# Prachet-Dev-Singh/DenseCLIP_Vit_multimodal

Measured on AMD Instinct MI355X. Metric: images/sec (fwd+bwd) ViT-B/16 DenseCLIP @1024x2048, higher is better.
Workload: dtype bf16

## Files before the change

### denseclip_vit_multimodal_amd/csrc/gemm.hip

```cpp
#include <mutex>
#include <type_traits>

#include "common.h"

namespace {

constexpr int BM = 128, BN = 128, BK = 64;
constexpr int TILE_BYTES = 128 * BK * 2;
constexpr int STAGE_BYTES = 2 * TILE_BYTES;
constexpr int EP_LD = 68;
constexpr int SMEM_BYTES = 4 * 64 * EP_LD * 4 > 2 * STAGE_BYTES ? 4 * 64 * EP_LD * 4 : 2 * STAGE_BYTES;

template <typename T>
__device__ __forceinline__ void store8(T* p, const float* v, bool full, int rem) {
    if (full) {
        if constexpr (sizeof(T) == 4) {
            f32x4 a = {v[0], v[1], v[2], v[3]}, b = {v[4], v[5], v[6], v[7]};
            *(f32x4*)p = a;
            *(f32x4*)(p + 4) = b;
        } else {
            typedef T t8 __attribute__((ext_vector_type(8)));
            t8 x;
#pragma unroll
            for (int e = 0; e < 8; ++e) x[e] = (T)v[e];
// ... 1581 lines not shown
    const int HW = g.H * g.W;
    const float invHW = 1.0f / (float)HW, invW = 1.0f / (float)g.W;
#pragma unroll
    for (int i = 0; i < ROWS_INST; ++i) {
        const int inst = wave * ROWS_INST + i;
        int m = m0 + inst * (64 / CPR) + lane / CPR;
        m = m < M ? m : M - 1;
        const int b = fdiv(m, HW, invHW);
        const int p = m - b * HW;
        const int y = fdiv(p, g.W, invW);
        R.y[i] = y;
        R.x[i] = p - y * g.W;
        R.base[i] = (int64_t)b * g.bstride + g.off + (int64_t)p * g.ld;
    }
}

template <typename T, int ROWS_INST, int BKT>
__device__ __forceinline__ void stage_conv_rows(const T* __restrict__ X, const T* __restrict__ zero,
                                                const ConvRows<ROWS_INST, BKT>& R, const PixGeo g, int Cin, int dir,
                                                int k0, char* lds, int wave, int lane) {
    constexpr int CPR = BKT / 8;
    const int tap = k0 / Cin, ci = k0 - tap * Cin;
    const int dy = (tap / 3 - 1) * dir, dx = (tap % 3 - 1) * dir;
    const int64_t shift = ((int64_t)dy * g.W + dx) * g.ld + ci;
#pragma unroll
    for (int i = 0; i < ROWS_INST; ++i) {
        const int inst = wave * ROWS_INST + i;
        const int r = inst * (64 / CPR) + lane / CPR;
        const int c = (lane % CPR) ^ big_sw<BKT>(r);
        const int yy = R.y[i] + dy, xx = R.x[i] + dx;
        const bool ok = yy >= 0 && yy < g.H && xx >= 0 && xx < g.W;
        const T* src = ok ? X + R.base[i] + shift + c * 8 : zero + c * 8;
        __builtin_amdgcn_global_load_lds((const void*)src, LDS_PTR(lds + inst * 1024), 16, 0, 0);
    }
}

template <typename T, int ROWS_INST, int BKT>
__device__ __forceinline__ void stage_conv_rows_buf(const T* X, uint32_t xbytes, const ConvRows<ROWS_INST, BKT>& R,
                                                    const PixGeo g, int Cin, int dir, int k0, char* lds, int wave,
                                                    int lane) {
#if defined(__HIP_DEVICE_COMPILE__)
    constexpr int CPR = BKT / 8;
    const rsrc_t rs = make_rsrc(X, xbytes);
    const int tap = k0 / Cin, ci = k0 - tap * Cin;
    const int dy = (tap / 3 - 1) * dir, dx = (tap % 3 - 1) * dir;
    const int shift = (int)((((int64_t)dy * g.W + dx) * g.ld + ci) * (int64_t)sizeof(T));
#pragma unroll
    for (int i = 0; i < ROWS_INST; ++i) {
        const int inst = wave * ROWS_INST + i;
        const int r = inst * (64 / CPR) + lane / CPR;
        const int c = (lane % CPR) ^ big_sw<BKT>(r);
        const int yy = R.y[i] + dy, xx = R.x[i] + dx;
        const bool ok = yy >= 0 && yy < g.H && xx >= 0 && xx < g.W;
        const uint32_t voff = ok ? (uint32_t)((int64_t)R.base[i] * (int64_t)sizeof(T) + shift + c * 16) : 0xFFFFFFF0u;
        __builtin_amdgcn_raw_ptr_buffer_load_lds(rs, LDS_PTR(lds + inst * 1024), 16, voff, 0, 0, 0);
    }
#endif
}

template <typename T, int EPI, typename OutT, int BM, int BN, int WM, int WN, int STAGES>
__global__ __launch_bounds__(64 * WM * WN, 1) void conv_nt_kernel(
    const T* __restrict__ X, const T* __restrict__ zero, PixGeo g, int Cin, int dir, const T* __restrict__ Bw,
    int64_t ldb, int M, int N, int tiles_m, int tiles_n, const void* __restrict__ aux, int64_t ld_aux,
    void* __restrict__ C, int64_t ldc, int map_hw, int map_gap, int map_off, uint32_t xbytes) {
    constexpr int BKT = 64;
    typedef BigCfg<BM, BN, WM, WN, STAGES, BKT> Cfg;
    typedef typename Mfma<T>::frag frag;
    __shared__ __attribute__((aligned(16))) char smem[Cfg::SMEM];
    const int lane = threadIdx.x & 63;
    const int wave = threadIdx.x >> 6;
    const int wm = wave / WN, wn = wave % WN;
    const int l16 = lane & 15, lq = lane >> 4;

    const int t = xcd_remap(blockIdx.x, tiles_m * tiles_n);
    const int m0 = (t / tiles_n) * BM;
    const int n0 = (t % tiles_n) * BN;
    const int nk = 9 * Cin / BKT;

    ConvRows<Cfg::A_INST, BKT> R;
    conv_rows_init<T, Cfg::A_INST, BKT>(R, g, M, m0, wave, lane);
    f32x4 acc[Cfg::NB][Cfg::MB];
#pragma unroll
    for (int i = 0; i < Cfg::NB; ++i)
#pragma unroll
        for (int j = 0; j < Cfg::MB; ++j) acc[i][j] = f32x4{0.f, 0.f, 0.f, 0.f};

    uint32_t vb[Cfg::B_INST];
    rows_voff<T, Cfg::B_INST, BKT>(ldb, n0, N, wave, lane, vb);
    const uint32_t bbytes = (uint32_t)((int64_t)N * ldb * sizeof(T));
    auto stage = [&](int kt, int slot) {
        char* base = smem + slot * Cfg::STAGE_BYTES;
        if (xbytes) stage_conv_rows_buf<T, Cfg::A_INST, BKT>(X, xbytes, R, g, Cin, dir, kt * BKT, base, wave, lane);
        else stage_conv_rows<T, Cfg::A_INST, BKT>(X, zero, R, g, Cin, dir, kt * BKT, base, wave, lane);
        stage_rows_buf<T, Cfg::B_INST>(Bw, bbytes, vb, (uint32_t)(kt * BKT * sizeof(T)), base + Cfg::A_BYTES, wave);
    };
#pragma unroll
    for (int s = 0; s < STAGES - 1; ++s)
        if (s < nk) stage(s, s);
    for (int kt = 0; kt < nk; ++kt) {
        if (kt + STAGES - 2 <= nk - 1) wait_vmcnt<Cfg::G * (STAGES - 2)>();
        else wait_vmcnt<0>();
        __builtin_amdgcn_s_barrier();
        __builtin_amdgcn_sched_barrier(0);
        if (kt + STAGES - 1 < nk) stage(kt + STAGES - 1, (kt + STAGES - 1) % STAGES);
        const char* At = smem + (kt % STAGES) * Cfg::STAGE_BYTES;
        const char* Bt = At + Cfg::A_BYTES;
#pragma unroll
        for (int ks = 0; ks < BKT / 32; ++ks) {
            frag fb[Cfg::NB], fa[Cfg::MB];
            const int ch = ks * 4 + lq;
#pragma unroll
            for (int i = 0; i < Cfg::NB; ++i) fb[i] = big_frag<T, BKT>(Bt, wn * Cfg::WTN + i * 16 + l16, ch);
#pragma unroll
            for (int j = 0; j < Cfg::MB; ++j) fa[j] = big_frag<T, BKT>(At, wm * Cfg::WTM + j * 16 + l16, ch);
#pragma unroll
            for (int j = 0; j < Cfg::MB; ++j)
#pragma unroll
                for (int i = 0; i < Cfg::NB; ++i) acc[i][j] = Mfma16<T>::mma(fb[i], fa[j], acc[i][j]);
        }
        __builtin_amdgcn_sched_barrier(0);
    }
    big_epilogue<T, EPI, OutT, Cfg>(acc, smem, M, N, m0 + wm * Cfg::WTM, n0 + wn * Cfg::WTN, nullptr, aux, ld_aux, C,
                                     ldc, nullptr, 0, 0, 1.0f, map_hw, map_gap, map_off);
}

template <typename T, bool AD = false>
__device__ __forceinline__ void stage_tile_tn_conv(const T* __restrict__ X, const T* __restrict__ zero, const PixGeo g,
                                                   int tap, int ci0, int k0, int krows, char* lds_tile, int wave,
                                                   int lane) {
    const int HW = g.H * g.W;
    const float invHW = 1.0f / (float)HW, invW = 1.0f / (float)g.W;
    const int dy = tap / 3 - 1, dx = tap % 3 - 1;
#pragma unroll
    for (int i = 0; i < 4; ++i) {
        const int inst = wave * 4 + i;
        const int r = inst * 4 + (lane >> 4);
        const int pc = lane & 15;
        const int c = pc ^ ((r & 3) << 2);
        int m = k0 + r;
        const bool in_k = m < krows;
        m = in_k ? m : krows - 1;
        const int b = fdiv(m, HW, invHW);
        const int p = m - b * HW;
        const int y = fdiv(p, g.W, invW);
        const int yy = y + dy, xx = p - y * g.W + dx;
        const bool ok = in_k && yy >= 0 && yy < g.H && xx >= 0 && xx < g.W;
        const T* src = ok ? X + (int64_t)b * g.bstride + g.off + ((int64_t)yy * g.W + xx) * g.ld + ci0 + c * 8
                          : zero + (c & 7) * 8;
        if constexpr (AD) glds16_asm(src, lds_tile + inst * 1024);
        else __builtin_amdgcn_global_load_lds((const void*)src, LDS_PTR(lds_tile + inst * 1024), 16, 0, 0);
    }
}

template <typename T, bool AD = false>
__global__ __launch_bounds__(256, 2) void conv_wgrad_kernel(const T* __restrict__ dY, int64_t ldy,
                                                            const T* __restrict__ X, const T* __restrict__ zero,
                                                            PixGeo g, int Cin, int M, int N, int Kpix, int k_chunk,
                                                            int tiles_m, int tiles_n, float* __restrict__ C,
                                                            int64_t slab) {
    __shared__ __attribute__((aligned(16))) char smem[SMEM_BYTES];
    const int lane = threadIdx.x & 63;
    const int wave = threadIdx.x >> 6;
    const int wm = wave >> 1, wn = wave & 1;
    const int t = xcd_remap(blockIdx.x, tiles_m * tiles_n);
    const int m0 = (t / tiles_n) * BM;
    const int n0 = (t % tiles_n) * BN;
    const int tap = n0 / Cin, ci0 = n0 - tap * Cin;
    const int kbeg = blockIdx.y * k_chunk;
    int nk = k_chunk / BK;
    if (kbeg + nk * BK > Kpix) nk = (Kpix - kbeg + BK - 1) / BK;
    nk = nk < 0 ? 0 : nk;

    f32x16 acc[2][2];
#pragma unroll
    for (int i = 0; i < 2; ++i)
#pragma unroll
        for (int j = 0; j < 2; ++j)
#pragma unroll
            for (int e = 0; e < 16; ++e) acc[i][j][e] = 0.f;
    if (nk > 0) {
        stage_tile_tn<T>(dY, ldy, kbeg, Kpix, m0, M, smem, wave, lane);
        stage_tile_tn_conv<T>(X, zero, g, tap, ci0, kbeg, Kpix, smem + TILE_BYTES, wave, lane);
    }
    __syncthreads();
    for (int kt = 0; kt < nk; ++kt) {
        const int cur = kt & 1;
        const char* At = smem + cur * STAGE_BYTES;
        const char* Bt = At + TILE_BYTES;
        const int k0 = kbeg + kt * BK;
        if (kt + 1 < nk) {
            char* nxt = smem + (cur ^ 1) * STAGE_BYTES;
            stage_tile_tn<T, AD>(dY, ldy, k0 + BK, Kpix, m0, M, nxt, wave, lane);
            stage_tile_tn_conv<T, AD>(X, zero, g, tap, ci0, k0 + BK, Kpix, nxt + TILE_BYTES, wave, lane);
        }
#pragma unroll
        for (int s = 0; s < 4; ++s) {
            typename Mfma<T>::frag fa[2], fb[2];
#pragma unroll
            for (int i = 0; i < 2; ++i) fa[i] = tr_frag_tn<T>(Bt, s, wn * 64 + i * 32, lane);
#pragma unroll
            for (int j = 0; j < 2; ++j) fb[j] = tr_frag_tn<T>(At, s, wm * 64 + j * 32, lane);
#pragma unroll
            for (int i = 0; i < 2; ++i)
#pragma unroll
                for (int j = 0; j < 2; ++j) acc[i][j] = Mfma<T>::mma(fa[i], fb[j], acc[i][j]);
        }
        if constexpr (AD) {
            wait_vmcnt<0>();
            __builtin_amdgcn_s_barrier();
        } else {
            __syncthreads();
        }
    }
    if constexpr (AD) __syncthreads();
    gemm_epilogue<T, DCLIP_EPI_SPLITK, float>(acc, smem, M, N, m0, n0, nullptr, nullptr, 0, C, N, nullptr, 0, slab,
                                               1.0f);
}

const void* conv_zero_row() {
    static void* z = nullptr;
    if (!z) {
        if (hipMalloc(&z, 256) != hipSuccess) return nullptr;
        if (hipMemset(z, 0, 256) != hipSuccess) return nullptr;
    }
    return z;
}

float* tail_scratch(size_t floats) {
    static float* buf = nullptr;
    static size_t cap = 0;
    if (floats > cap) {
        if (buf) (void)hipFree(buf);
        buf = nullptr;
        cap = 0;
        if (hipMalloc(&buf, floats * sizeof(float)) != hipSuccess) return nullptr;
        cap = floats;
    }
    return buf;
}

template <typename T, int EPI, typename OutT>
__global__ __launch_bounds__(512) void gemm_tail16_kernel(const T* __restrict__ A, int64_t lda, const T* __restrict__ B,
                                                          int64_t ldb, int mt, int N, int K, int m0,
                                                          const float* __restrict__ bias, const void* __restrict__ aux,
                                                          int64_t ld_aux, void* __restrict__ C, int64_t ldc,
                                                          void* __restrict__ C2, int64_t ldc2, Alpha alpha_arg) {
    typedef typename Mfma<T>::frag frag;
    __shared__ float red[8][16][68];
    const int lane = threadIdx.x & 63, wave = threadIdx.x >> 6;
    const int l16 = lane & 15, lq = lane >> 4;
    const int n0 = blockIdx.x * 64;
    const int ks = K / 8, kbeg = wave * ks;
    const bool rowok = l16 < mt;
    const T* arow = A + (int64_t)(rowok ? l16 : 0) * lda + kbeg + 8 * lq;
    const T* brow = B + (int64_t)(n0 + l16) * ldb + kbeg + 8 * lq;
    f32x4 acc[4];
#pragma unroll
    for (int i = 0; i < 4; ++i) acc[i] = f32x4{0.f, 0.f, 0.f, 0.f};
    frag zf;
#pragma unroll
    for (int j = 0; j < 8; ++j) zf[j] = (T)0.f;
#pragma unroll 4
    for (int k = 0; k < ks; k += 32) {
        const frag a = rowok ? *(const frag*)(arow + k) : zf;
        frag b[4];
#pragma unroll
        for (int i = 0; i < 4; ++i) b[i] = *(const frag*)(brow + (int64_t)16 * i * ldb + k);
#pragma unroll
        for (int i = 0; i < 4; ++i) acc[i] = Mfma16<T>::mma(a, b[i], acc[i]);
    }
#pragma unroll
    for (int i = 0; i < 4; ++i)
#pragma unroll
        for (int e = 0; e < 4; ++e) red[wave][4 * lq + e][16 * i + l16] = acc[i][e];
    __syncthreads();
    const int t = threadIdx.x;
    if (t < 128) {
        const int r = t >> 3, cb = (t & 7) * 8;
        if (r < mt) {
            const float alpha = alpha_arg.get();
            float v[8];
#pragma unroll
            for (int e = 0; e < 8; ++e) {
                float sum = 0.f;
#pragma unroll
                for (int w = 0; w < 8; ++w) sum += red[w][r][cb + e];
                v[e] = sum * alpha;
            }
            epi_row8<T, EPI, OutT>(v, m0 + r, n0 + cb, N, bias, aux, ld_aux, C, ldc, C2, ldc2, 0);
        }
    }
}

template <typename T, int EPI, typename OutT>
__global__ __launch_bounds__(1024) void gemm_tail16x16_kernel(const T* __restrict__ A, int64_t lda,
                                                              const T* __restrict__ B, int64_t ldb, int mt, int N,
                                                              int W, int IT, int m0, const float* __restrict__ bias,
                                                              const void* __restrict__ aux, int64_t ld_aux,
                                                              void* __restrict__ C, int64_t ldc, void* __restrict__ C2,
                                                              int64_t ldc2, Alpha alpha_arg) {
    typedef typename Mfma<T>::frag frag;
    constexpr int ITMAX = 6;
    __shared__ float red[16][16][17];
    const int lane = threadIdx.x & 63, wave = threadIdx.x >> 6;
    const int l16 = lane & 15, lq = lane >> 4;
    const int n0 = blockIdx.x * 16;
    const int t = threadIdx.x;
    const int er = t >> 1, ecb = (t & 1) * 8;
    const bool epi = t < 2 * mt;
    float bv[8], pre[8];
#pragma unroll
    for (int e = 0; e < 8; ++e) bv[e] = pre[e] = 0.f;
    if (epi) {
        const int nb = n0 + ecb;
        if (bias != nullptr && EPI != DCLIP_EPI_GELU_BWD) load8<float>(bias + nb, bv, true, 8);
        if constexpr (EPI == DCLIP_EPI_STORE_SCALED) load8<float>((const float*)aux + nb, pre, true, 8);
        if constexpr (EPI == DCLIP_EPI_RESIDUAL)
            load8<float>((const float*)aux + (int64_t)(m0 + er) * ld_aux + nb, pre, true, 8);
        if constexpr (EPI == DCLIP_EPI_GELU_BWD) load8<T>((const T*)aux + (int64_t)(m0 + er) * ld_aux + nb, pre, true, 8);
    }
    const bool rowok = l16 < mt;
    const int kbeg = wave * IT * 32;
    const T* arow = A + (int64_t)(rowok ? l16 : 0) * lda + kbeg + 8 * lq;
    const T* brow = B + (int64_t)(n0 + l16) * ldb + kbeg + 8 * lq;
    frag zf;
#pragma unroll
    for (int j = 0; j < 8; ++j) zf[j] = (T)0.f;
    frag a[ITMAX], b[ITMAX];
#pragma unroll
    for (int it = 0; it < ITMAX; ++it) {
        if (it < IT) {
            a[it] = rowok ? *(const frag*)(arow + 32 * it) : zf;
            b[it] = *(const frag*)(brow + 32 * it);
        }
    }
    f32x4 acc = f32x4{0.f, 0.f, 0.f, 0.f};
#pragma unroll
    for (int it = 0; it < ITMAX; ++it)
        if (it < IT) acc = Mfma16<T>::mma(a[it], b[it], acc);
#pragma unroll
    for (int e = 0; e < 4; ++e) red[wave][4 * lq + e][l16] = acc[e];
    __syncthreads();
    if (epi) {
        const float alpha = alpha_arg.get();
        float v[8];
#pragma unroll
        for (int e = 0; e < 8; ++e) {
            float sum = 0.f;
            for (int w = 0; w < W; ++w) sum += red[w][er][ecb + e];
            v[e] = sum * alpha + bv[e];
        }
        const int64_t m = m0 + er;
        const int nb = n0 + ecb;
        if constexpr (EPI == DCLIP_EPI_STORE) {
            store8<OutT>((OutT*)C + m * ldc + nb, v, true, 8);
        } else if constexpr (EPI == DCLIP_EPI_STORE_SCALED) {
#pragma unroll
            for (int e = 0; e < 8; ++e) v[e] *= pre[e];
            store8<OutT>((OutT*)C + m * ldc + nb, v, true, 8);
        } else if constexpr (EPI == DCLIP_EPI_GELU) {
            float g[8];
#pragma unroll
            for (int e = 0; e < 8; ++e) {
                v[e] = (float)(OutT)v[e];
                g[e] = quick_gelu(v[e]);
            }
            if (C != nullptr) store8<OutT>((OutT*)C + m * ldc + nb, v, true, 8);
            store8<OutT>((OutT*)C2 + m * ldc2 + nb, g, true, 8);
        } else if constexpr (EPI == DCLIP_EPI_RESIDUAL) {
// ... 393 lines not shown
                             void* ws, void* C, int64_t ldc, float* colsum_a, void* stream) {
    const Alpha alpha(alpha_v, alpha_ptr);
    DCLIP_HOST_CHECK(ab_dt == DCLIP_BF16 || ab_dt == DCLIP_F16, "dclip_gemm_tn: operands must be f16/bf16");
    DCLIP_HOST_CHECK(M > 0 && N > 0 && K > 0 && M % 8 == 0 && N % 8 == 0,
                     "dclip_gemm_tn: M, N must be positive multiples of 8 (M=%lld N=%lld)", (long long)M, (long long)N);
    DCLIP_HOST_CHECK(splits >= 1 && K_pad >= K && K_pad % (BK * splits) == 0,
                     "dclip_gemm_tn: K_pad must be >= K and a multiple of 64*splits");
    DCLIP_HOST_CHECK(lda >= M && ldb >= N && lda % 8 == 0 && ldb % 8 == 0, "dclip_gemm_tn: bad leading dims");
    DCLIP_HOST_CHECK(((uintptr_t)A % 16) == 0 && ((uintptr_t)B % 16) == 0, "dclip_gemm_tn: A/B must be 16-byte aligned");
    DCLIP_HOST_CHECK(epilogue == DCLIP_EPI_STORE || epilogue == DCLIP_EPI_SPLITK,
                     "dclip_gemm_tn: epilogue must be STORE or SPLITK (f32 output)");
    DCLIP_HOST_CHECK(epilogue == DCLIP_EPI_STORE ? splits == 1 : ws != nullptr,
                     "dclip_gemm_tn: STORE needs splits == 1; SPLITK needs a workspace of splits*(M*N + M) f32");
    DCLIP_HOST_CHECK(ldc % 4 == 0, "dclip_gemm_tn: ldc %% 4 != 0");
    DCLIP_HOST_CHECK(K * lda * 2 < (1ll << 32) && K * ldb * 2 < (1ll << 32),
                     "dclip_gemm_tn: operands must stay below 4 GiB (buffer-load staging)");
    hipStream_t st = (hipStream_t)stream;
    const int tiles_m = (int)((M + BM - 1) / BM), tiles_n = (int)((N + BN - 1) / BN);
    const int k_chunk = (int)(K_pad / splits);
    dim3 grid(tiles_m * tiles_n, splits);
    const int tn_opt = dclip_option(DCLIP_OPT_GEMM_TN_TILE);
    const bool tn_pf = dclip_option(DCLIP_OPT_GEMM_KLOOP) == 1;
    const bool big = tn_opt != 1 && M >= 256 && N >= 256;
    const bool fused_cs =
        colsum_a && big && tn_opt != 2 && tn_opt != 3 && dclip_option(DCLIP_OPT_GEMM_TN_COLSUM) != 1;
    float* cs_sep = (colsum_a && !fused_cs && epilogue == DCLIP_EPI_SPLITK) ? (float*)ws + (int64_t)splits * M * N
                                                                           : nullptr;
    if (colsum_a && !fused_cs) {
        const int64_t rpb = cs_sep != nullptr ? K_pad / splits : K;
        dim3 cg((unsigned)((M + 63) / 64), (unsigned)(cs_sep != nullptr ? splits : 1));
        if (ab_dt == DCLIP_BF16)
            colsum_kernel<bf16><<<cg, 256, 0, st>>>((const bf16*)A, lda, K, (int)M, rpb, alpha, colsum_a, cs_sep);
        else colsum_kernel<f16><<<cg, 256, 0, st>>>((const f16*)A, lda, K, (int)M, rpb, alpha, colsum_a, cs_sep);
    }
#define TN_LAUNCH_V(T, EPI, OUT, AD)                                                                              \
    gemm_tn_kernel<T, EPI, float, AD><<<grid, 256, 0, st>>>((const T*)A, lda, (const T*)B, ldb, (int)M, (int)N,    \
                                                            (int)K, k_chunk, tiles_m, tiles_n, nullptr, OUT,         \
                                                            EPI == DCLIP_EPI_SPLITK ? N : ldc, (int64_t)M * N, alpha)
#define TN_LAUNCH(T, EPI, OUT)                                                                                    \
    do {                                                                                                          \
        if (tn_opt == 5) TN_LAUNCH_V(T, EPI, OUT, false);                                                         \
        else TN_LAUNCH_V(T, EPI, OUT, true);                                                                      \
    } while (0)
#define TN_BIG_V(T, EPI, OUT, BKT, STG, CS, NW, ...)                                                           \
    gemm_tn_big_kernel<T, EPI, BKT, STG, CS, NW, ##__VA_ARGS__><<<dim3(tm2 * tn2 * splits), 64 * NW, 0, st>>>( \
        (const T*)A, lda, (const T*)B, ldb, (int)M, (int)N, (int)K, k_chunk, tm2, tn2, OUT,                     \
        EPI == DCLIP_EPI_SPLITK ? N : ldc, (int64_t)M * N, alpha, EPI == DCLIP_EPI_SPLITK ? cs_part : colsum_a)
#define TN_BIG(T, EPI, OUT)                                                                                    \
    do {                                                                                                       \
        if (tn_opt == 2) TN_BIG_V(T, EPI, OUT, 32, 4, false, 8);                                               \
        else if (tn_opt == 3) TN_BIG_V(T, EPI, OUT, 32, 5, false, 8);                                          \
        else if (tn_opt == 4 && fused_cs) TN_BIG_V(T, EPI, OUT, 64, 2, true, 4);                               \
        else if (tn_opt == 4) TN_BIG_V(T, EPI, OUT, 64, 2, false, 4);                                          \
        else if (tn_opt == 5 && fused_cs) TN_BIG_V(T, EPI, OUT, 64, 2, true, 8);                               \
        else if (tn_opt == 5) TN_BIG_V(T, EPI, OUT, 64, 2, false, 8);                                          \
        else if (fused_cs && tn_pf) TN_BIG_V(T, EPI, OUT, 64, 2, true, 8, true, true);                         \
        else if (tn_pf) TN_BIG_V(T, EPI, OUT, 64, 2, false, 8, true, true);                                    \
        else if (fused_cs) TN_BIG_V(T, EPI, OUT, 64, 2, true, 8, false, true);                                 \
        else TN_BIG_V(T, EPI, OUT, 64, 2, false, 8, false, true);                                              \
    } while (0)
    const int tm2 = (int)((M + 255) / 256), tn2 = (int)((N + 255) / 256);
    float* cs_part = (fused_cs && epilogue == DCLIP_EPI_SPLITK) ? (float*)ws + (int64_t)splits * M * N : cs_sep;
    if (epilogue == DCLIP_EPI_STORE) {
        DCLIP_HOST_CHECK(bias == nullptr, "dclip_gemm_tn: bias only with SPLITK");
        if (big) {
            if (ab_dt == DCLIP_BF16) TN_BIG(bf16, DCLIP_EPI_STORE, C);
            else TN_BIG(f16, DCLIP_EPI_STORE, C);
        } else {
            if (ab_dt == DCLIP_BF16) TN_LAUNCH(bf16, DCLIP_EPI_STORE, C);
            else TN_LAUNCH(f16, DCLIP_EPI_STORE, C);
        }
    } else {
        if (big) {
            if (ab_dt == DCLIP_BF16) TN_BIG(bf16, DCLIP_EPI_SPLITK, ws);
            else TN_BIG(f16, DCLIP_EPI_SPLITK, ws);
        } else {
            if (ab_dt == DCLIP_BF16) TN_LAUNCH(bf16, DCLIP_EPI_SPLITK, ws);
            else TN_LAUNCH(f16, DCLIP_EPI_SPLITK, ws);
        }
        const int64_t total4 = M * (N / 4);
        int blocks = (int)((total4 + 255) / 256);
        blocks = blocks > 4096 ? 4096 : blocks;
        splitk_reduce_kernel<<<blocks, 256, 0, st>>>((const float*)ws, splits, M * N, (int)M, (int)N, bias,
                                                     (float*)C, ldc, cs_part, colsum_a);
    }
#undef TN_LAUNCH
#undef TN_LAUNCH_V
#undef TN_BIG
#undef TN_BIG_V
    DCLIP_LAUNCH_CHECK();
    return 0;
}

extern "C" int dclip_conv3x3(int mode, int ab_dt, const void* X, int64_t x_bstride, int64_t x_off, int64_t x_ld,
                             int B, int H, int W, int Cin, const void* Wt, int Nout, void* out, int out_dt,
                             int64_t out_ld, int out_gap, int out_off, int accumulate, void* stream) {
    DCLIP_HOST_CHECK(ab_dt == DCLIP_BF16 || ab_dt == DCLIP_F16, "dclip_conv3x3: operands must be f16/bf16");
    DCLIP_HOST_CHECK(mode == 0 || mode == 1, "dclip_conv3x3: mode 0 (forward) or 1 (input gradient)");
    DCLIP_HOST_CHECK(B > 0 && H > 0 && W > 0 && Cin > 0 && Nout > 0 && Cin % 64 == 0 && Nout % 8 == 0,
                     "dclip_conv3x3: Cin %% 64 == 0 and Nout %% 8 == 0 required (Cin=%d Nout=%d)", Cin, Nout);
    DCLIP_HOST_CHECK((int64_t)B * H * W < (1ll << 24), "dclip_conv3x3: too many pixels");
    DCLIP_HOST_CHECK(x_ld % 8 == 0 && x_bstride % 8 == 0 && x_off % 8 == 0 && x_ld >= Cin,
                     "dclip_conv3x3: input strides must be multiples of 8 elements");
    DCLIP_HOST_CHECK(((uintptr_t)X % 16) == 0 && ((uintptr_t)Wt % 16) == 0, "dclip_conv3x3: unaligned operands");
    DCLIP_HOST_CHECK(out_dt == ab_dt || out_dt == DCLIP_F32, "dclip_conv3x3: output must be f32 or the operand dtype");
    DCLIP_HOST_CHECK(!accumulate || out_dt == DCLIP_F32, "dclip_conv3x3: accumulate needs an f32 output");
    const void* zero = conv_zero_row();
    DCLIP_HOST_CHECK(zero != nullptr, "dclip_conv3x3: zero row allocation failed");
    hipStream_t st = (hipStream_t)stream;
    const PixGeo g{x_bstride, x_off, (int)x_ld, H, W};
    const int M = B * H * W;
    const int dir = mode == 0 ? 1 : -1;
    constexpr int TBM = 256, TBN = 128;
    const int tiles_m = (M + TBM - 1) / TBM, tiles_n = (Nout + TBN - 1) / TBN;
    const int map_hw = out_gap ? H * W : 0;
    const int64_t xext = ((int64_t)(B - 1) * x_bstride + x_off + (int64_t)H * W * x_ld) * 2;
    const uint32_t xbytes = xext < (1ll << 32) - 4096 ? (uint32_t)xext : 0u;
#define CONV_LAUNCH(T, EPI, OUTT)                                                                                    \
    conv_nt_kernel<T, EPI, OUTT, TBM, TBN, 4, 2, 3><<<tiles_m * tiles_n, 512, 0, st>>>(                             \
        (const T*)X, (const T*)zero, g, Cin, dir, (const T*)Wt, 9 * (int64_t)Cin, M, Nout, tiles_m, tiles_n, out,    \
        out_ld, out, out_ld, map_hw, out_gap, out_off, xbytes)
    if (ab_dt == DCLIP_BF16) {
        if (accumulate) CONV_LAUNCH(bf16, DCLIP_EPI_RESIDUAL, float);
        else if (out_dt == DCLIP_F32) CONV_LAUNCH(bf16, DCLIP_EPI_STORE, float);
        else CONV_LAUNCH(bf16, DCLIP_EPI_STORE, bf16);
    } else {
        if (accumulate) CONV_LAUNCH(f16, DCLIP_EPI_RESIDUAL, float);
        else if (out_dt == DCLIP_F32) CONV_LAUNCH(f16, DCLIP_EPI_STORE, float);
        else CONV_LAUNCH(f16, DCLIP_EPI_STORE, f16);
    }
#undef CONV_LAUNCH
    DCLIP_LAUNCH_CHECK();
    return 0;
}

extern "C" int dclip_conv3x3_wgrad(int ab_dt, const void* dY, int64_t ldy, int Nout, const void* X, int64_t x_bstride,
                                   int64_t x_off, int64_t x_ld, int B, int H, int W, int Cin, float* dW, void* ws,
                                   int splits, int oihw, const float* alpha_ptr, void* stream) {
    DCLIP_HOST_CHECK(ab_dt == DCLIP_BF16 || ab_dt == DCLIP_F16, "dclip_conv3x3_wgrad: operands must be f16/bf16");
    DCLIP_HOST_CHECK(Cin % 128 == 0 && Nout % 8 == 0 && Nout > 0 && ldy % 8 == 0 && ldy >= Nout,
                     "dclip_conv3x3_wgrad: Cin %% 128 == 0 and Nout %% 8 == 0 required");
    DCLIP_HOST_CHECK(x_ld % 8 == 0 && x_bstride % 8 == 0 && x_off % 8 == 0, "dclip_conv3x3_wgrad: bad strides");
    DCLIP_HOST_CHECK(splits >= 1 && ws != nullptr, "dclip_conv3x3_wgrad: workspace of splits * Nout * 9 * Cin f32");
    DCLIP_HOST_CHECK((int64_t)B * H * W < (1ll << 24), "dclip_conv3x3_wgrad: too many pixels");
    const void* zero = conv_zero_row();
    DCLIP_HOST_CHECK(zero != nullptr, "dclip_conv3x3_wgrad: zero row allocation failed");
    hipStream_t st = (hipStream_t)stream;
    const PixGeo g{x_bstride, x_off, (int)x_ld, H, W};
    const int Kpix = B * H * W;
    const int N = 9 * Cin;
    const int kp = (Kpix + 64 * splits - 1) / (64 * splits) * 64;
    const int tiles_m = (Nout + BM - 1) / BM, tiles_n = N / BN;
    dim3 grid(tiles_m * tiles_n, splits);
#define WG_LAUNCH(T, AD)                                                                                        \
    conv_wgrad_kernel<T, AD><<<grid, 256, 0, st>>>((const T*)dY, ldy, (const T*)X, (const T*)zero, g, Cin, Nout, N, \
                                                   Kpix, kp, tiles_m, tiles_n, (float*)ws, (int64_t)Nout * N)
    const bool ad = dclip_option(DCLIP_OPT_GEMM_TN_TILE) != 5;
    if (ab_dt == DCLIP_BF16) {
        if (ad) WG_LAUNCH(bf16, true);
        else WG_LAUNCH(bf16, false);
    } else {
        if (ad) WG_LAUNCH(f16, true);
        else WG_LAUNCH(f16, false);
    }
#undef WG_LAUNCH
    if (oihw || alpha_ptr != nullptr) {
        const int64_t total = (int64_t)Nout * Cin;
        const int blocks = (int)((total + 255) / 256 > 4096 ? 4096 : (total + 255) / 256);
        if (oihw) {
            conv_wgrad_reduce_oihw_kernel<<<blocks, 256, 0, st>>>((const float*)ws, splits, (int64_t)Nout * N, Nout, Cin,
                                                                  Alpha(1.f, alpha_ptr), dW);
            DCLIP_LAUNCH_CHECK();
            return 0;
        }
        DCLIP_HOST_CHECK(false, "dclip_conv3x3_wgrad: alpha_ptr needs the OIHW output");
    }
    const int64_t total4 = (int64_t)Nout * (N / 4);
    int blocks = (int)((total4 + 255) / 256);
    blocks = blocks > 4096 ? 4096 : blocks;
    splitk_reduce_kernel<<<blocks, 256, 0, st>>>((const float*)ws, splits, (int64_t)Nout * N, Nout, N, nullptr, dW,
                                                 N);
    DCLIP_LAUNCH_CHECK();
    return 0;
}
```

Measured before the change: 65.08.

## Carry pixel coordinates across K-steps in conv3x3 wgrad; add row-reuse kernel

The default conv3x3 weight-gradient path now keeps per-row pixel index, x coordinate and batch base in registers and advances them incrementally each K-step. This replaces the per-tile integer divisions used to compute im2col addresses. Separately, an opt-in kernel (option 7) builds one 17-row X tile per dy and derives all three dx taps from row-shifted LDS reads, masking image-edge columns. It uses a 3-stage pipeline with 512 threads. The carried path adds a vmcnt wait after the first stage, and its while-loop wrap only handles small strides cleanly.

```diff
diff --git a/denseclip_vit_multimodal_amd/csrc/gemm.hip b/denseclip_vit_multimodal_amd/csrc/gemm.hip
--- a/denseclip_vit_multimodal_amd/csrc/gemm.hip
+++ b/denseclip_vit_multimodal_amd/csrc/gemm.hip
@@ -1757,7 +1757,51 @@
     }
 }
 
-template <typename T, bool AD = false>
+struct TapRows {
+    int p[4], x[4];
+    int64_t base[4];
+};
+__device__ __forceinline__ void tap_rows_init(TapRows& R, const PixGeo g, int k0, int wave, int lane) {
+    const int HW = g.H * g.W;
+#pragma unroll
+    for (int i = 0; i < 4; ++i) {
+        const int m = k0 + (wave * 4 + i) * 4 + (lane >> 4);
+        const int b = m / HW;
+        R.p[i] = m - b * HW;
+        R.x[i] = R.p[i] % g.W;
+        R.base[i] = (int64_t)b * g.bstride + g.off;
+    }
+}
+template <typename T>
+__device__ __forceinline__ void stage_tile_tn_conv_carried(const T* __restrict__ X, const T* __restrict__ zero,
+                                                           const PixGeo g, int tap, int ci0, int k0, int krows,
+                                                           TapRows& R, char* lds_tile, int wave, int lane) {
+    const int HW = g.H * g.W, xstep = BK % g.W;
+    const int dy = tap / 3 - 1, dx = tap % 3 - 1;
+    const int plo = dy < 0 ? g.W : 0, phi = dy > 0 ? HW - g.W : HW;
+    const int xlo = dx < 0 ? 1 : 0, xhi = dx > 0 ? g.W - 1 : g.W;
+    const int shift = dy * g.W + dx;
+#pragma unroll
+    for (int i = 0; i < 4; ++i) {
+        const int inst = wave * 4 + i;
+        const int r = inst * 4 + (lane >> 4);
+        const int pc = lane & 15;
+        const int c = pc ^ ((r & 3) << 2);
+        const int p = R.p[i], x = R.x[i];
+        const bool ok = (k0 + r < krows) & (p >= plo) & (p < phi) & (x >= xlo) & (x < xhi);
+        const T* in = X + R.base[i] + (int64_t)(p + shift) * g.ld + ci0 + c * 8;
+        const T* src = ok ? in : zero + (c & 7) * 8;
+        glds16_asm(src, lds_tile + inst * 1024);
+        R.p[i] = p + BK;
+        R.x[i] = x + xstep >= g.W ? x + xstep - g.W : x + xstep;
+        while (R.p[i] >= HW) {
+            R.p[i] -= HW;
+            R.base[i] += g.bstride;
+        }
+    }
+}
+
+template <typename T, bool AD = false, bool CARRY = false>
 __global__ __launch_bounds__(256, 2) void conv_wgrad_kernel(const T* __restrict__ dY, int64_t ldy,
                                                             const T* __restrict__ X, const T* __restrict__ zero,
                                                             PixGeo g, int Cin, int M, int N, int Kpix, int k_chunk,
@@ -1783,9 +1827,16 @@
         for (int j = 0; j < 2; ++j)
 #pragma unroll
             for (int e = 0; e < 16; ++e) acc[i][j][e] = 0.f;
+    TapRows R;
+    if constexpr (CARRY) tap_rows_init(R, g, kbeg, wave, lane);
     if (nk > 0) {
         stage_tile_tn<T>(dY, ldy, kbeg, Kpix, m0, M, smem, wave, lane);
-        stage_tile_tn_conv<T>(X, zero, g, tap, ci0, kbeg, Kpix, smem + TILE_BYTES, wave, lane);
+        if constexpr (CARRY) {
+            stage_tile_tn_conv_carried<T>(X, zero, g, tap, ci0, kbeg, Kpix, R, smem + TILE_BYTES, wave, lane);
+            wait_vmcnt<0>();
+        } else {
+            stage_tile_tn_conv<T>(X, zero, g, tap, ci0, kbeg, Kpix, smem + TILE_BYTES, wave, lane);
+        }
     }
     __syncthreads();
     for (int kt = 0; kt < nk; ++kt) {
@@ -1796,7 +1847,9 @@
         if (kt + 1 < nk) {
             char* nxt = smem + (cur ^ 1) * STAGE_BYTES;
             stage_tile_tn<T, AD>(dY, ldy, k0 + BK, Kpix, m0, M, nxt, wave, lane);
-            stage_tile_tn_conv<T, AD>(X, zero, g, tap, ci0, k0 + BK, Kpix, nxt + TILE_BYTES, wave, lane);
+            if constexpr (CARRY)
+                stage_tile_tn_conv_carried<T>(X, zero, g, tap, ci0, k0 + BK, Kpix, R, nxt + TILE_BYTES, wave, lane);
+            else stage_tile_tn_conv<T, AD>(X, zero, g, tap, ci0, k0 + BK, Kpix, nxt + TILE_BYTES, wave, lane);
         }
 #pragma unroll
         for (int s = 0; s < 4; ++s) {
@@ -1820,6 +1873,194 @@
     if constexpr (AD) __syncthreads();
     gemm_epilogue<T, DCLIP_EPI_SPLITK, float>(acc, smem, M, N, m0, n0, nullptr, nullptr, 0, C, N, nullptr, 0, slab,
                                                1.0f);
+}
+
+constexpr bool CONV_WGRAD_ROWS_DEFAULT = false;
+constexpr bool CONV_WGRAD_CARRY_DEFAULT = true;
+constexpr int RW_A_BYTES = 64 * 256;
+constexpr int RW_X_PIECES = 17;
+constexpr int RW_STAGE_BYTES = RW_A_BYTES + RW_X_PIECES * 1024;
+constexpr int RW_STAGES = 3;
+constexpr int RW_EP_LD = 36;
+constexpr int RW_SMEM = RW_STAGES * RW_STAGE_BYTES > 8 * 64 * RW_EP_LD * 4 ? RW_STAGES * RW_STAGE_BYTES
+                                                                          : 8 * 64 * RW_EP_LD * 4;
+
+template <typename T>
+__device__ __forceinline__ typename Mfma<T>::frag tr_frag_rows(const char* img, int row0, int col_base, int lane) {
+    const int i = lane & 15, q = i >> 2, p = i & 3, g = lane >> 4, h = lane >> 5;
+    const int row = row0 + 8 * h + q;
+    const int col = col_base + (g & 1) * 16 + 4 * p;
+    typedef __attribute__((address_space(3))) i16x4 lds_i16x4;
+    auto off = [](int r, int c) { return r * 256 + (((c >> 3) ^ ((r & 3) << 2)) << 4) + ((c & 7) << 1); };
+    i16x4 lo = __builtin_amdgcn_ds_read_tr16_b64_v4i16((lds_i16x4*)(img + off(row, col)));
+    i16x4 hi = __builtin_amdgcn_ds_read_tr16_b64_v4i16((lds_i16x4*)(img + off(row + 4, col)));
+    typedef short s8 __attribute__((ext_vector_type(8)));
+    s8 v = __builtin_shufflevector(lo, hi, 0, 1, 2, 3, 4, 5, 6, 7);
+    return __builtin_bit_cast(typename Mfma<T>::frag, v);
+}
+
+template <typename F>
+__device__ __forceinline__ F zero_frag_rows(F f, uint32_t bits) {
+    typedef uint32_t u4 __attribute__((ext_vector_type(4)));
+    u4 v = __builtin_bit_cast(u4, f);
+#pragma unroll
+    for (int d = 0; d < 4; ++d) {
+        const uint32_t keep = ((bits >> (2 * d)) & 1u ? 0u : 0x0000FFFFu) | ((bits >> (2 * d + 1)) & 1u ? 0u : 0xFFFF0000u);
+        v[d] &= keep;
+    }
+    return __builtin_bit_cast(F, v);
+}
+
+template <typename T, int MJ>
+__global__ __launch_bounds__(512, 1) void conv_wgrad_rows_kernel(const T* __restrict__ dY, int64_t ldy,
+                                                                 const T* __restrict__ X, const T* __restrict__ zero,
+                                                                 PixGeo g, int Cin, int M, int N, int Kpix, int k_chunk,
+                                                                 int tiles_m, float* __restrict__ C, int64_t slab) {
+    typedef typename Mfma<T>::frag frag;
+    __shared__ __attribute__((aligned(16))) char smem[RW_SMEM];
+    const int lane = threadIdx.x & 63;
+    const int wave = __builtin_amdgcn_readfirstlane(threadIdx.x >> 6);
+    const int wm = wave >> 2, wq = wave & 3;
+    const int h = lane >> 5;
+    const int cb = Cin / 128;
+    const int t = xcd_remap(blockIdx.x, tiles_m * 3 * cb);
+    const int m0 = (t / (3 * cb)) * (64 * MJ);
+    const int rem = t % (3 * cb);
+    const int dy = rem / cb - 1, ci0 = (rem % cb) * 128;
+    const int W = g.W, HW = g.H * g.W;
+    const int kbeg = blockIdx.y * k_chunk;
+    int nk = k_chunk / BK;
+    if (kbeg + nk * BK > Kpix) nk = (Kpix - kbeg + BK - 1) / BK;
+    nk = nk < 0 ? 0 : nk;
+
+    f32x16 acc[3][MJ];
+#pragma unroll
+    for (int d = 0; d < 3; ++d)
+#pragma unroll
+        for (int j = 0; j < MJ; ++j)
+#pragma unroll
+            for (int e = 0; e < 16; ++e) acc[d][j][e] = 0.f;
+
+    const int lrow = lane >> 4, pc = lane & 15;
+    int xp[3];
+    int64_t xbase[3];
+#pragma unroll
+    for (int i = 0; i < 3; ++i) {
+        const int piece = i < 2 ? wave * 2 + i : 16;
+        const int m = kbeg - 1 + piece * 4 + lrow;
+        const int b = m >= 0 ? m / HW : -1;
+        xp[i] = m - b * HW;
+        xbase[i] = (int64_t)b * g.bstride + g.off;
+    }
+    int ks = kbeg;
+    const int plo = dy < 0 ? W : 0, phi = dy > 0 ? HW - W : HW;
+    auto stage = [&](int slot) {
+        char* At = smem + slot * RW_STAGE_BYTES;
+        char* Xt = At + RW_A_BYTES;
+#pragma unroll
+        for (int i = 0; i < 2; ++i) {
+            const int inst = wave * 2 + i;
+            const int r = inst * 4 + lrow;
+            const int c = pc ^ ((r & 3) << 2);
+            int gr = ks + r;
+            gr = gr < Kpix ? gr : Kpix - 1;
+            int gc = m0 + c * 8;
+            gc = gc + 8 <= M ? gc : M - 8;
+            glds16_asm(dY + (int64_t)gr * ldy + gc, At + inst * 1024);
+        }
+#pragma unroll
+        for (int i = 0; i < 3; ++i) {
+            const int piece = i < 2 ? wave * 2 + i : 16;
+            if (i < 2 || wave == 0) {
+                const int lr = piece * 4 + lrow;
+                const int c = pc ^ ((lr & 3) << 2);
+                const int m = ks - 1 + lr;
+                const bool ok = (m >= 0) & (m < Kpix) & (xp[i] >= plo) & (xp[i] < phi);
+                const T* in = X + xbase[i] + (int64_t)(xp[i] + dy * W) * g.ld + ci0 + c * 8;
+                const T* src = ok ? in : zero + (c & 7) * 8;
+                glds16_asm(src, Xt + piece * 1024);
+            }
+            xp[i] += BK;
+            while (xp[i] >= HW) {
+                xp[i] -= HW;
+                xbase[i] += g.bstride;
+            }
+        }
+        ks += BK;
+    };
+
+    if (nk > 0) stage(0);
+    if (nk > 1) stage(1);
+    int xk = kbeg % W;
+    const int xstep = BK % W;
+    int cur = 0, nxt = 2;
+    const int mc0 = (MJ == 2 ? 64 : 32) * wm;
+    for (int kt = 0; kt < nk; ++kt) {
+        if (kt + 1 < nk) wait_vmcnt<4>();
+        else wait_vmcnt<0>();
+        __builtin_amdgcn_s_barrier();
+        __builtin_amdgcn_sched_barrier(0);
+        if (kt + 2 < nk) stage(nxt);
+        const char* At = smem + cur * RW_STAGE_BYTES;
+        const char* Xt = At + RW_A_BYTES;
+        uint64_t mL = 0, mR = 0;
+        for (int r = xk == 0 ? 0 : W - xk; r <= BK; r += W) {
+            if (r < BK) mL |= 1ull << r;
+            if (r > 0) mR |= 1ull << (r - 1);
+        }
+        const bool edge = (mL | mR) != 0;
+#pragma unroll
+        for (int s = 0; s < 4; ++s) {
+            frag fa[3], fb[MJ];
+#pragma unroll
+            for (int j = 0; j < MJ; ++j) fb[j] = tr_frag_rows<T>(At, 16 * s, mc0 + 32 * j, lane);
+#pragma unroll
+            for (int d = 0; d < 3; ++d) fa[d] = tr_frag_rows<T>(Xt, 16 * s + d, 32 * wq, lane);
+            if (edge) {
+                fa[0] = zero_frag_rows(fa[0], (uint32_t)(mL >> (16 * s + 8 * h)) & 0xFFu);
+                fa[2] = zero_frag_rows(fa[2], (uint32_t)(mR >> (16 * s + 8 * h)) & 0xFFu);
+            }
+#pragma unroll
+            for (int d = 0; d < 3; ++d)
+#pragma unroll
+                for (int j = 0; j < MJ; ++j) acc[d][j] = Mfma<T>::mma(fa[d], fb[j], acc[d][j]);
+        }
+        __builtin_amdgcn_sched_barrier(0);
+        xk += xstep;
+        xk = xk >= W ? xk - W : xk;
+        cur = cur == 2 ? 0 : cur + 1;
+        nxt = nxt == 2 ? 0 : nxt + 1;
+    }
+    __syncthreads();
+
+    float* ep = (float*)smem + wave * (64 * RW_EP_LD);
+    const int l32 = lane & 31;
+    const int c4 = (lane & 7) * 4;
+    float* Cs = C + blockIdx.y * slab;
+#pragma unroll
+    for (int d = 0; d < 3; ++d) {
+#pragma unroll
+        for (int j = 0; j < MJ; ++j)
+#pragma unroll
+            for (int q = 0; q < 4; ++q) {
+                f32x4 v;
+#pragma unroll
+                for (int e = 0; e < 4; ++e) v[e] = acc[d][j][4 * q + e];
+                *(f32x4*)(ep + (j * 32 + l32) * RW_EP_LD + q * 8 + h * 4) = v;
+            }
+        __builtin_amdgcn_s_waitcnt(0xc07f);
+        __builtin_amdgcn_wave_barrier();
+        const int n = ((dy + 1) * 3 + d) * Cin + ci0 + 32 * wq + c4;
+#pragma unroll
+        for (int it = 0; it < 4 * MJ; ++it) {
+            const int r = it * 8 + (lane >> 3);
+            const int m = m0 + mc0 + r;
+            const f32x4 v = *(const f32x4*)(ep + r * RW_EP_LD + c4);
+            if (m < M) *(f32x4*)(Cs + (int64_t)m * N + n) = v;
+        }
+        __builtin_amdgcn_s_waitcnt(0xc07f);
+        __builtin_amdgcn_wave_barrier();
+    }
 }
 
 const void* conv_zero_row() {
@@ -2519,16 +2760,33 @@
     const int kp = (Kpix + 64 * splits - 1) / (64 * splits) * 64;
     const int tiles_m = (Nout + BM - 1) / BM, tiles_n = N / BN;
     dim3 grid(tiles_m * tiles_n, splits);
-#define WG_LAUNCH(T, AD)                                                                                        \
-    conv_wgrad_kernel<T, AD><<<grid, 256, 0, st>>>((const T*)dY, ldy, (const T*)X, (const T*)zero, g, Cin, Nout, N, \
-                                                   Kpix, kp, tiles_m, tiles_n, (float*)ws, (int64_t)Nout * N)
-    const bool ad = dclip_option(DCLIP_OPT_GEMM_TN_TILE) != 5;
-    if (ab_dt == DCLIP_BF16) {
-        if (ad) WG_LAUNCH(bf16, true);
-        else WG_LAUNCH(bf16, false);
+#define WG_LAUNCH(T, AD, CARRY)                                                                                 \
+    conv_wgrad_kernel<T, AD, CARRY><<<grid, 256, 0, st>>>((const T*)dY, ldy, (const T*)X, (const T*)zero, g, Cin, Nout, \
+                                                          N, Kpix, kp, tiles_m, tiles_n, (float*)ws, (int64_t)Nout * N)
+    const int wg_opt = dclip_option(DCLIP_OPT_GEMM_TN_TILE);
+    if (wg_opt == 7 || (CONV_WGRAD_ROWS_DEFAULT && wg_opt == 0)) {
+        const int mj = Nout <= 64 ? 1 : 2;
+        const int tm = (Nout + 64 * mj - 1) / (64 * mj);
+        dim3 rgrid(tm * 3 * (Cin / 128), splits);
+#define WGR_LAUNCH(T, MJ)                                                                                            \
+    conv_wgrad_rows_kernel<T, MJ><<<rgrid, 512, 0, st>>>((const T*)dY, ldy, (const T*)X, (const T*)zero, g, Cin, Nout, N, \
+                                                        Kpix, kp, tm, (float*)ws, (int64_t)Nout * N)
+        if (ab_dt == DCLIP_BF16) {
+            if (mj == 1) WGR_LAUNCH(bf16, 1);
+            else WGR_LAUNCH(bf16, 2);
+        } else {
+            if (mj == 1) WGR_LAUNCH(f16, 1);
+            else WGR_LAUNCH(f16, 2);
+        }
+#undef WGR_LAUNCH
+    } else if (ab_dt == DCLIP_BF16) {
+        if (wg_opt == 5) WG_LAUNCH(bf16, false, false);
+        else if (wg_opt != 8 && (wg_opt == 6 || !CONV_WGRAD_CARRY_DEFAULT)) WG_LAUNCH(bf16, true, false);
+        else WG_LAUNCH(bf16, true, true);
     } else {
-        if (ad) WG_LAUNCH(f16, true);
-        else WG_LAUNCH(f16, false);
+        if (wg_opt == 5) WG_LAUNCH(f16, false, false);
+        else if (wg_opt != 8 && (wg_opt == 6 || !CONV_WGRAD_CARRY_DEFAULT)) WG_LAUNCH(f16, true, false);
+        else WG_LAUNCH(f16, true, true);
     }
 #undef WG_LAUNCH
     if (oihw || alpha_ptr != nullptr) {
```

Result: no change. 65.47, median of 3 (+0.6%).
